# interactiveaudiolab/emphases

Hardware: AMD Instinct MI355X
Metric: utterances/s (10 s @16 kHz) whole-node (higher is better)
Workload: dtype f32; 1 GPU; 64 synthetic 10 s 16 kHz utterances per GPU, conv config, random word alignments, ragged batch with per-utterance (B=1) semantics (BASELINE.json configs[1]); utterances_per_gpu=64, frames_per_gpu=64000, words_per_gpu=1882, conv_tile=64, launch=hipGraph replay, batches_in_flight=2, parallelism=utterance-sharded x1, exchange=none (one rank)

## Files before the change

### emphases_amd/csrc/decoder.hip

```cpp
#include <math.h>
#include <stdint.h>

#include <type_traits>

#include "common.h"

namespace emph {

typedef float f32x4 __attribute__((ext_vector_type(4)));

constexpr int kWindow = 64;
constexpr int kLeadCols = 4;
constexpr int kActStride = 80;

__device__ __forceinline__ float activate_word(float x, int act) {
    switch (act) {
        case EMPH_ACT_RELU: return fmaxf(x, 0.f);
        case EMPH_ACT_GELU: return 0.5f * x * (1.f + erff(x * 0.70710678118654752440f));
        case EMPH_ACT_SILU: return x / (1.f + expf(-x));
        case EMPH_ACT_LEAKY_RELU: return x > 0.f ? x : 0.01f * x;
        default: return x;
    }
}

#ifndef EMPH_DECODER_LOADERS
#define EMPH_DECODER_LOADERS 4
#endif
constexpr int kLoaderWaves = EMPH_DECODER_LOADERS;

template <int KS, int MT>
__global__ __launch_bounds__(64 * (8 + kLoaderWaves)) void word_decoder_kernel(
    const float* __restrict__ x, int64_t ldx, const int32_t* __restrict__ tiles,
    int block, int halo, int channels, const float* __restrict__ packs,
    const float* __restrict__ biases, int layers, int act, int chunk_trips,
    const float* __restrict__ out_weight, const float* __restrict__ out_bias,
    int out_kernel, int post, float* __restrict__ logits, float* __restrict__ scores) {
    extern __shared__ __align__(16) float lds[];
    const int m_tiles = channels >> 4;
    const int threads = blockDim.x;
    const int waves = threads >> 6;
    const int compute_waves = waves - kLoaderWaves;
    const int buffer_floats = channels * kActStride;
    float* partial = lds + 2 * channels * kActStride;
    float* bias_lds = partial + waves * kWindow;
    float* out_lds = bias_lds + layers * channels;
    float* ring = lds + ((2 * channels * kActStride + waves * kWindow + layers * channels +
                          channels * out_kernel + 1 + 3) & ~3);
    const int lane = threadIdx.x & 63;
    const int wave = __builtin_amdgcn_readfirstlane(threadIdx.x >> 6);
    const int kk = lane >> 4;
    const int col = lane & 15;

    const Tile span = load_tile(tiles, blockIdx.x);
    const int reach = 32 - halo;
    const bool halves = span.count > 32 && span.count <= 2 * reach;
    const bool second = halves && span.first != 0;
    const bool single = span.count <= kWindow && !halves;
    if (single && span.first != 0) return;
    const int half = (span.count + 1) >> 1;
    const int first_out = halves ? (second ? half : 0) : span.first;
    const int last_out = halves   ? (second ? span.count : half)
                         : single ? span.count
                                  : min(span.first + block, span.count);
    const int start = halves ? (second ? span.count - 32 : 0) : single ? 0 : span.first - halo;
    const bool narrow = halves || (single && span.count <= 32);

    constexpr int HALO = (KS - 1) / 2;
    constexpr int kTripFloats = 4 * KS;
    const int trips = channels >> 4;
    const int trip_floats = m_tiles * 64 * kTripFloats;
    const int chunks_per_layer = (trips + chunk_trips - 1) / chunk_trips;
    const int total_chunks = layers * chunks_per_layer;
    const int chunk_floats = chunk_trips * trip_floats;
    auto request = [&](int q) {
        const int layer = q / chunks_per_layer;
        const int first = (q - layer * chunks_per_layer) * chunk_trips;
        const int quads = min(chunk_trips, trips - first) * (trip_floats >> 2);
        const float* source =
            packs + (static_cast<int64_t>(layer) * trips + first) * trip_floats;
        float* target = ring + (q & 1) * chunk_floats;
        for (int base = 64 * (wave - compute_waves); base < quads;
             base += 64 * kLoaderWaves)
            __builtin_amdgcn_global_load_lds(
                (const __attribute__((address_space(1))) void*)(source + 4 * (base + lane)),
                (__attribute__((address_space(3))) void*)(target + 4 * base), 16, 0, 0);
    };
    const bool loader = wave >= compute_waves;
    if (total_chunks > 0 && loader) request(0);

    for (int index = threadIdx.x; index < channels * (kActStride / 4); index += threads) {
        const int c = index / (kActStride / 4);
        const int quad = index - c * (kActStride / 4);
        float4 value = make_float4(0.f, 0.f, 0.f, 0.f);
        const int p = 4 * quad - kLeadCols;
        if (p >= 0 && p < kWindow) {
            const int word = start + p;
            const float* source = x + static_cast<int64_t>(c) * ldx + span.offset + word;
            if (word >= 0 && word + 3 < span.count &&
                (reinterpret_cast<uintptr_t>(source) & 15) == 0) {
                value = *reinterpret_cast<const float4*>(source);
            } else {
                if (word >= 0 && word < span.count) value.x = source[0];
                if (word + 1 >= 0 && word + 1 < span.count) value.y = source[1];
                if (word + 2 >= 0 && word + 2 < span.count) value.z = source[2];
                if (word + 3 >= 0 && word + 3 < span.count) value.w = source[3];
            }
        }
        reinterpret_cast<float4*>(lds)[index] = value;
        reinterpret_cast<float4*>(lds + buffer_floats)[index] =
            make_float4(0.f, 0.f, 0.f, 0.f);
    }
    for (int index = threadIdx.x; index < layers * channels; index += threads)
        bias_lds[index] = biases[index];
    for (int index = threadIdx.x; index <= channels * out_kernel; index += threads)
        out_lds[index] = index < channels * out_kernel ? out_weight[index] : out_bias[0];

    if (loader) {
        for (int q = 0; q < total_chunks; ++q) {
            __builtin_amdgcn_s_waitcnt(0x0F70);
            __syncthreads();
            if (q + 1 < total_chunks) request(q + 1);
        }
    }

    const int n_tile = narrow ? (wave & 1) : (wave & 3);
    const int part = narrow ? (wave >> 1) : (wave >> 2);
    const int split = (m_tiles + 1) >> 1;
    const int m_begin = narrow ? (m_tiles * part + 3) >> 2 : (part ? split : 0);
    const int m_end = narrow ? (m_tiles * (part + 1) + 3) >> 2 : (part ? m_tiles : split);
    const int m_count = m_end - m_begin;
    auto run_layers = [&](auto count_tag) {
        constexpr int COUNT = decltype(count_tag)::value;
        int buffer = 0;
        for (int layer = 0; layer < layers; ++layer) {
            const float* source = lds + buffer * buffer_floats;
            float* target = lds + (buffer ^ 1) * buffer_floats;
// ... 41 lines not shown
                    for (int tap = 0; tap < KS; ++tap)
#pragma unroll
                        for (int i = 0; i < COUNT; ++i) {
                            acc[i] = __builtin_amdgcn_mfma_f32_16x16x4f32(
                                a[i][(t * KS + tap) >> 2][(t * KS + tap) & 3], b[t][tap],
                                acc[i], 0, 0, 0);
                        }
#pragma unroll
                for (int k = 0; k < (COUNT + 4) * KS; ++k) {
                    __builtin_amdgcn_sched_group_barrier(0x008, 1, 0);
                    __builtin_amdgcn_sched_group_barrier(0x100, 1, 0);
                }
                __builtin_amdgcn_sched_barrier(0);
            };
            __syncthreads();
            if (kTwoSets) {
                issue(a_set[0], b_set[0], 0);
                for (int trip = 0; trip < trips; trip += 2) {
                    step(a_set[0], b_set[0], a_set[kTwoSets], b_set[kTwoSets], trip);
                    if (trip + 1 < trips)
                        step(a_set[kTwoSets], b_set[kTwoSets], a_set[0], b_set[0], trip + 1);
                }
            } else {
                for (int trip = 0; trip < trips; ++trip)
                    step(a_set[0], b_set[0], a_set[0], b_set[0], trip);
            }
            const float* bias = bias_lds + layer * channels + 16 * m_begin + 4 * kk;
            const int p = 16 * n_tile + col;
            const int word = start + p;
            const bool inside = word >= 0 && word < span.count;
            f32x4 value[COUNT];
#pragma unroll
            for (int i = 0; i < COUNT; ++i)
                value[i] = acc[i] + *reinterpret_cast<const f32x4*>(bias + 16 * i);
#define EMPH_APPLY(EXPRESSION)                                   \
    _Pragma("unroll") for (int i = 0; i < COUNT; ++i)            \
// ... 6 lines not shown
                case EMPH_ACT_GELU:
                    EMPH_APPLY(0.5f * v * (1.f + erff(v * 0.70710678118654752440f)));
                    break;
                case EMPH_ACT_SILU: EMPH_APPLY(v / (1.f + expf(-v))); break;
                case EMPH_ACT_LEAKY_RELU: EMPH_APPLY(v > 0.f ? v : 0.01f * v); break;
                default: break;
            }
#undef EMPH_APPLY
#pragma unroll
            for (int i = 0; i < COUNT; ++i)
#pragma unroll
                for (int r = 0; r < 4; ++r) {
                    const int c = 16 * (m_begin + i) + 4 * kk + r;
                    target[c * kActStride + kLeadCols + p] = inside ? value[i][r] : 0.f;
                }
            buffer ^= 1;
        }
    };
    if (!loader) {
        if (m_count >= 4 && MT >= 4) run_layers(std::integral_constant<int, MT >= 4 ? 4 : 1>{});
        else if (m_count == 3) run_layers(std::integral_constant<int, 3>{});
        else if (m_count == 2) run_layers(std::integral_constant<int, 2>{});
        else if (m_count == 1) run_layers(std::integral_constant<int, 1>{});
        else
            for (int q = 0; q < total_chunks; ++q) __syncthreads();
    }
    int current = layers & 1;
    __syncthreads();

    {
        const float* source = lds + current * buffer_floats;
        const int halo_out = (out_kernel - 1) / 2;
        float sum = 0.f;
        for (int c = wave; c < channels && !loader; c += compute_waves)
// ... 6 lines not shown
            float total = out_lds[channels * out_kernel];
            for (int w = 0; w < compute_waves; ++w) total += partial[w * kWindow + lane];
            const int word = start + lane;
            if (word >= first_out && word < last_out) {
                const int64_t column = span.offset + word;
                if (logits != nullptr) logits[column] = total;
                if (scores != nullptr) {
                    float value = total;
                    if (post == EMPH_POST_SIGMOID) value = 1.f / (1.f + expf(-total));
                    if (post == EMPH_POST_CLAMP01) value = fminf(fmaxf(total, 0.f), 1.f);
                    scores[column] = value;
                }
            }
        }
    }
}

}

using namespace emph;

extern "C" {

int64_t emph_word_decoder_pack_size(int32_t channels, int32_t kernel_size) {
    return static_cast<int64_t>(channels) * channels * kernel_size;
}

int emph_word_decoder_pack(const float* host_weight, int32_t channels, int32_t kernel_size,
                           float* host_pack) {
    EMPH_REQUIRE(host_weight && host_pack, EMPH_EINVAL,
// ... 46 lines not shown
    for (int segment = 0; segment < segments; ++segment) {
        const int64_t count = host_counts[segment];
        if (count <= 0) continue;
        if (count > 32 && count <= 2 * (32 - halo)) {
            emit(segment, 0);
            emit(segment, (count + 1) / 2);
        } else if (count <= kWindow) {
            emit(segment, 0);
        } else {
            for (int64_t first = 0; first < count; first += block) emit(segment, first);
        }
    }
    return total;
}

int emph_word_decoder(const float* x, int64_t ldx, const int32_t* tiles,
                      int32_t n_tiles, int32_t channels, const float* packs,
                      const float* biases, int32_t layers, int32_t kernel_size,
                      int32_t activation, const float* out_weight,
                      const float* out_bias, int32_t out_kernel_size, int32_t post,
                      float* logits, float* scores, void* stream) {
    if (n_tiles == 0) return EMPH_OK;
    EMPH_REQUIRE(x && tiles && out_weight && out_bias, EMPH_EINVAL,
                 "emph_word_decoder: null pointer");
    EMPH_REQUIRE(layers == 0 || (packs && biases), EMPH_EINVAL,
                 "emph_word_decoder: decoder weights are null");
    EMPH_REQUIRE(layers >= 0 && layers <= 16, EMPH_ERANGE,
                 "emph_word_decoder: %d layers", layers);
    EMPH_REQUIRE(channels >= 16 && channels <= 128 && channels % 16 == 0, EMPH_ERANGE,
                 "emph_word_decoder: channels %d not a multiple of 16 in 16..128",
                 channels);
    EMPH_REQUIRE(kernel_size == 1 || kernel_size == 3 || kernel_size == 5, EMPH_ERANGE,
                 "emph_word_decoder: kernel_size %d not in {1,3,5}", kernel_size);
    EMPH_REQUIRE(out_kernel_size >= 1 && out_kernel_size <= 7 && (out_kernel_size & 1),
                 EMPH_ERANGE, "emph_word_decoder: out_kernel_size %d", out_kernel_size);
    const int block = emph_word_decoder_block(layers, kernel_size, out_kernel_size);
    EMPH_REQUIRE(block >= 16, EMPH_ERANGE,
                 "emph_word_decoder: receptive field too wide for a 64-word window");
    const int halo = (kWindow - block) / 2;
    const int m_tiles = channels / 16;
    const int threads = 64 * (8 + kLoaderWaves);
    const size_t fixed_floats = (2 * channels * kActStride + (threads / 64) * kWindow +
                                 layers * channels + channels * out_kernel_size + 1 + 3) & ~3;
    size_t ring_budget = 156 * 1024 - fixed_floats * sizeof(float);
    const int trips = channels / 16;
    const size_t trip_bytes = static_cast<size_t>(m_tiles) * 64 * 4 * kernel_size * sizeof(float);
    int chunk_trips = static_cast<int>(ring_budget / 2 / trip_bytes);
    EMPH_REQUIRE(chunk_trips >= 1, EMPH_ERANGE,
                 "emph_word_decoder: no LDS left for the weight ring (%d channels, %d layers)",
                 channels, layers);
    if (chunk_trips > trips) chunk_trips = trips;
    const int pieces = (trips + chunk_trips - 1) / chunk_trips;
    chunk_trips = (trips + pieces - 1) / pieces;
    const size_t lds = fixed_floats * sizeof(float) + 2 * chunk_trips * trip_bytes;
    hipStream_t s = static_cast<hipStream_t>(stream);
#define EMPH_WORDS(KS)                                                              \
    do {                                                                            \
        auto kernel = m_tiles <= 6 ? word_decoder_kernel<KS, 3>                     \
                                   : word_decoder_kernel<KS, 4>;                    \
        static LdsReservation reserved[2];                                                     \
        if (int status = reserve_lds(reserved[m_tiles <= 6], reinterpret_cast<const void*>(kernel), lds,\
                                     "emph_word_decoder"))                                     \
            return status;                                                                     \
        EMPH_LAUNCH(kernel, dim3(n_tiles), dim3(threads), lds, s, x, ldx,     \
                           tiles, block, halo, channels, packs, biases, layers,      \
                           activation, chunk_trips, out_weight, out_bias,            \
                           out_kernel_size, post, logits, scores);                   \
    } while (0)
    switch (kernel_size) {
        case 1: EMPH_WORDS(1); break;
        case 3: EMPH_WORDS(3); break;
        default: EMPH_WORDS(5); break;
    }
#undef EMPH_WORDS
    return check_launch("emph_word_decoder");
}

}
```

### emphases_amd/csrc/forward.hip

```cpp
#include "common.h"

using namespace emph;

namespace emph {
__global__ __launch_bounds__(64) void launch_probe_kernel() {}
}

extern "C" {

int emph_launch_probe(void* stream) {
    EMPH_LAUNCH(launch_probe_kernel, dim3(1), dim3(64), 0, static_cast<hipStream_t>(stream));
    return check_launch("emph_launch_probe");
}

int64_t emph_prominence_workspace_floats(int32_t features, int32_t channels,
                                         int64_t ld_frames, int64_t ld_words,
                                         int32_t n_slots) {
    return (static_cast<int64_t>(features) + 2 * channels) * ld_frames +
           static_cast<int64_t>(channels) * (ld_words + n_slots);
}

int emph_prominence_forward(const emph_conv_model* model, const void* audio,
                            int32_t audio_format, const int64_t* seg,
                            const int32_t* frontend_tiles,
// ... 39 lines not shown
                 "emph_prominence_forward: word_sums needs conv_variant 1 and a sum / average "
                 "reduction");

    int status = emph_logmel(audio, audio_format, seg, frontend_tiles, n_frontend_tiles, m.table,
                             m.mel_start, m.mel_count, m.mel_offset, m.mel_values, m.mel_nnz,
                             features, ld_frames, 0, -1, nullptr, nullptr, m.normalize, stream);
    if (status) return status;
    auto conv = [&](const float* in, float* out, const float* pack, const float* bias, int c_in,
                    int activation) {
        return quad ? emph_conv1d_winograd4(in, ld_frames, out, ld_frames, pack, bias, c_in, c,
                                            activation, frame_tiles, n_frame_tiles, stream)
                    : emph_conv1d_winograd(in, ld_frames, out, ld_frames, pack, bias, c_in, c,
                                           activation, frame_tiles, n_frame_tiles, tile_n,
                                           stream);
    };
    const int64_t pack_floats =
        quad ? emph_conv_winograd4_pack_size(c, c) : emph_conv_winograd_pack_size(c, c);
    const bool stack = conv_spans != nullptr && quad && c == 80 && m.features == 80 &&
                       m.encoder_packs == m.input_pack + pack_floats &&
                       m.encoder_biases == m.input_bias + c &&
                       (m.activation == EMPH_ACT_RELU || m.activation == EMPH_ACT_NONE);
    if (stack) {
        const bool composed = m.compose != nullptr && m.encoder_layers >= 1;
        const int skip = composed ? 1 : 0;
        const int total = 1 + m.encoder_layers - skip;
        const int most = emph_conv_stack_max_layers();
        const int groups = (total + most - 1) / most;
        float* buffers[2] = {current, other};
        const float* in = features;
        int done = 0;
// ... 13 lines not shown
                               n_conv_spans, to_sums ? word_sums->slot_map : nullptr, stream)
                         : emph_conv1d_stack(in, ld_frames, out, to_sums ? c : ld_frames, packs,
                                             biases, size, relu, conv_spans, n_conv_spans,
                                             to_sums ? word_sums->slot_map : nullptr, stream);
            if (status) return status;
            in = out;
            done += size;
        }
        current = const_cast<float*>(in);
        status = fold ? emph_word_sums(sums, c, word_sums->terms, word_sums->first,
                                       word_sums->lengths, words, ld_words, c, ld_words,
                                       m.reduction, stream)
                      : emph_segment_reduce(current, ld_frames, bounds, words, ld_words, c, seg,
                                            word_segment, ld_words, m.reduction, stream);
        if (status) return status;
        return emph_word_decoder(words, ld_words, word_tiles, n_word_tiles, c, m.decoder_packs,
                                 m.decoder_biases, m.decoder_layers, m.decoder_kernel_size,
                                 m.activation, m.out_weight, m.out_bias, m.decoder_kernel_size,
                                 m.post, logits, scores, stream);
    }
    status = conv(features, current, m.input_pack, m.input_bias, m.features, EMPH_ACT_NONE);
    if (status) return status;
    for (int layer = 0; layer < m.encoder_layers; ++layer) {
        if (fold && layer == m.encoder_layers - 1) {
            status = emph_conv1d_winograd4_word_sums(
                current, ld_frames, sums, c, m.encoder_packs + layer * pack_floats,
                m.encoder_biases + static_cast<int64_t>(layer) * c, c, c, m.activation,
                frame_tiles, n_frame_tiles, word_sums->slot_map, stream);
            if (status) return status;
            break;
        }
        status = conv(current, other, m.encoder_packs + layer * pack_floats,
                      m.encoder_biases + static_cast<int64_t>(layer) * c, c, m.activation);
        if (status) return status;
        float* swap = current;
        current = other;
        other = swap;
    }
    status = fold ? emph_word_sums(sums, c, word_sums->terms, word_sums->first,
                                   word_sums->lengths, words, ld_words, c, ld_words,
                                   m.reduction, stream)
                  : emph_segment_reduce(current, ld_frames, bounds, words, ld_words, c, seg,
                                        word_segment, ld_words, m.reduction, stream);
    if (status) return status;
    return emph_word_decoder(words, ld_words, word_tiles, n_word_tiles, c, m.decoder_packs,
                             m.decoder_biases, m.decoder_layers, m.decoder_kernel_size,
                             m.activation, m.out_weight, m.out_bias, m.decoder_kernel_size,
                             m.post, logits, scores, stream);
}

}
```

### emphases_amd/engine.py

```python
import contextlib
import functools
import os
import ctypes
import threading

import numpy as np
import torch

from . import config as cfg
from . import melbasis
from . import runtime
from . import weights as weights_module

FRONTEND_BLOCK = None
PRECISIONS = {'f32': (0, 0, 0), 'bf16x3': (2, 32, 3), 'bf16x3_fast': (2, 32, 2),
              'bf16x6': (0, 3, 3)}
ATTENTION_BLOCK = 64
ATTENTION_GROUP = 256
GROUPED_FROM = ATTENTION_GROUP // 2
FUSED_WORDS = 64
EVERYTHING = 1 << 30
SHORT, LONG = (0, GROUPED_FROM - 1), (GROUPED_FROM, EVERYTHING)
FEW_WORDS, MANY_WORDS = (0, FUSED_WORDS), (FUSED_WORDS + 1, EVERYTHING)
WORD_TILE = 16
# ... 122 lines not shown
        self.mel_values = to(basis.values)
        self.mel_nnz = int(basis.values.size)
        self.a_weights = to(a_weighting())

        self.input_layer = _Conv(
            state['input_layer.weight'], state['input_layer.bias'], dev,
            winograd)
        self.frame_encoder = self._stack('frame_encoder')
        self.word_decoder = self._stack('word_decoder') \
            if config.has_decoder else None
        self.output_weight = to(state['output_layer.weight'])
        self.output_bias = to(state['output_layer.bias'])
        self.fused_words = config.architecture == 'convolution' or \
            not config.has_decoder
        self.word_block = WORD_TILE
        if self.fused_words:
            layers = self.word_decoder if config.has_decoder else []
            self.decoder_layers = len(layers)
            self.decoder_packs = torch.from_numpy(np.concatenate([
                runtime.word_decoder_pack(l.weight) for l in layers])).to(dev) \
                if layers else None
            self.decoder_biases = torch.cat([l.bias for l in layers]) \
                if layers else None
            self.word_block = int(self.lib.emph_word_decoder_block(
                self.decoder_layers, config.decoder_kernel_size,
                config.decoder_kernel_size))
            self.decoder_tiles = (runtime.AXIS_DECODER, (
                self.decoder_layers, config.decoder_kernel_size,
                config.decoder_kernel_size))
        if config.architecture == 'transformer':
            self.position = to(weights_module.positional_encoding(
                cfg.MAX_POSITIONS, config.channels))
            self.position_rows = self.position.t().contiguous()
        self.word_transformer = None
        if config.architecture == 'transformer' and config.has_decoder and \
                config.channels in (64, 80) and config.heads == 2 and all(
                    tuple(state[f'word_decoder.model.layers.{i}.{name}.weight']
                          .shape) == (config.channels, config.channels)
# ... 88 lines not shown
            post=runtime.POSTPROCESS[config.loss],
            normalize=int(config.normalize), mel_nnz=self.mel_nnz,
            conv_variant=int(self.quad),
            table=pointer(self.table), mel_start=pointer(self.mel_start),
            mel_count=pointer(self.mel_count),
            mel_offset=pointer(self.mel_offset),
            mel_values=pointer(self.mel_values),
            input_pack=pointer(input_pack),
            input_bias=pointer(input_bias),
            encoder_packs=pointer(self._encoder_packs),
            encoder_biases=pointer(self._encoder_biases),
            decoder_packs=pointer(self.decoder_packs),
            decoder_biases=pointer(self.decoder_biases),
            out_weight=pointer(self.output_weight),
            out_bias=pointer(self.output_bias),
            compose=pointer(self._compose_pack if self.stack else None))

    def _stack(self, prefix):
        config, state, dev = self.config, self.state, self.device
        layers = []
        if config.architecture == 'convolution':
            for i in range(config.layers):
                layers.append(_Conv(
                    state[f'{prefix}.{2 * i}.weight'],
                    state[f'{prefix}.{2 * i}.bias'], dev,
                    self.winograd and prefix == 'frame_encoder'))
            return layers
        channels = config.channels
        to = lambda a: torch.from_numpy(np.ascontiguousarray(a)).to(dev)
        for i in range(config.layers):
            p = f'{prefix}.model.layers.{i}.'
# ... 889 lines not shown
            logits[at:at + size].copy_(
                part_logits[batch.LEAD:batch.LEAD + size])
        return scores, logits

    def _word_stage(self, wa, plan, meta, logits, scores):
        config = self.config
        channels = config.channels
        ld_w = plan.ld_words
        words = runtime.AXIS_WORDS
        table = meta['table'][0]
        if self.fused_words:
            tiles, size = meta[('tiles',) + self.decoder_tiles]
            with self._timed('word_decoder', 2. * channels * (
                    channels * config.decoder_kernel_size * self.decoder_layers
                    + config.decoder_kernel_size) * plan.total_words):
                runtime.check(self.lib.emph_word_decoder(
                    wa.data_ptr(), ld_w, tiles.data_ptr(),
                    size // runtime.TILE_FIELDS, channels,
                    None if self.decoder_packs is None
                    else self.decoder_packs.data_ptr(),
                    None if self.decoder_biases is None
                    else self.decoder_biases.data_ptr(),
                    self.decoder_layers, config.decoder_kernel_size,
                    runtime.ACTIVATIONS[config.activation],
                    self.output_weight.data_ptr(), self.output_bias.data_ptr(),
                    config.decoder_kernel_size,
                    runtime.POSTPROCESS[config.loss], logits.data_ptr(),
                    scores.data_ptr(), runtime.stream()), 'emph_word_decoder')
            return scores, logits
        wb = self._buffer('words_b', channels, ld_w)
        decoded = self._stack_forward(
            self.word_decoder, wa, wb, ld_w, plan, meta, words,
            self.word_block, 'words')
        with self._timed('output_layer'):
            runtime.check(self.lib.emph_output_layer(
# ... 79 lines not shown
```

### emphases_amd/runtime.py

```python
import ctypes
import os

import numpy as np
import torch

HERE = os.path.dirname(os.path.abspath(__file__))
LIBRARY_PATH = os.path.join(HERE, 'libemphases_hip.so')
ABI_VERSION = 39

SEG_FIELDS = 8
TILE_FIELDS = 4
(SEG_AUDIO_OFF, SEG_AUDIO_LEN, SEG_START, SEG_LENGTH, SEG_FRAME_OFF,
 SEG_FRAMES, SEG_WORD_OFF, SEG_WORDS) = range(8)
AXIS_FRAMES, AXIS_WORDS = 0, 1
AXIS_DECODER = 2
ACTIVATIONS = {None: 0, 'none': 0, 'relu': 1, 'gelu': 2, 'silu': 3,
               'leaky_relu': 4}
REDUCTIONS = {'sum': 0, 'average': 1, 'max': 2, 'center': 3}
POSTPROCESS = {None: 0, 'bce': 1, 'mse': 2}
BCE_FORMS = {'bce': 0, 'mse': 1}
AUDIO_F32, AUDIO_PCM16 = 0, 1
SPREAD_IDENTITY, SPREAD_LOG2 = 0, 1
(METRIC_COUNT, METRIC_BCE, METRIC_SQUARED_ERROR, METRIC_COVARIANCE,
 METRIC_SUM_PREDICTED, METRIC_SUMSQ_PREDICTED, METRIC_SUM_TARGET,
# ... 126 lines not shown
        _ptr, _ptr, _i64, _ptr, _ptr]),
    'emph_plan_word_sums': (_i64, [
        _ptr, _ptr, _ptr, _i32, _ptr, _ptr, _i64, _ptr, _i64, _i64, _i64,
        _ptr, _ptr, _ptr, _ptr, _i64, _ptr]),
    'emph_gather_columns': (_c.c_int, [
        _ptr, _i64, _ptr, _i64, _i32, _ptr, _i32, _ptr]),
    'emph_collate': (_c.c_int, [
        _ptr, _i64, _ptr, _i64, _ptr, _i32, _i32, _i64, _i64, _ptr, _ptr,
        _ptr]),
    'emph_unpack_rows': (_c.c_int, [_ptr, _i64, _ptr, _i32, _ptr, _ptr]),
    'emph_word_decoder_block': (_i32, [_i32, _i32, _i32]),
    'emph_word_decoder_tiles': (_i32, [_ptr, _ptr, _i32, _i32, _i32, _i32, _ptr]),
    'emph_word_decoder_pack_size': (_i64, [_i32, _i32]),
    'emph_word_decoder_pack': (_c.c_int, [_ptr, _i32, _i32, _ptr]),
    'emph_word_decoder': (_c.c_int, [
        _ptr, _i64, _ptr, _i32, _i32, _ptr, _ptr, _i32, _i32, _i32, _ptr, _ptr,
        _i32, _i32, _ptr, _ptr, _ptr]),
    'emph_add_position': (_c.c_int, [
        _ptr, _i64, _ptr, _i32, _i32, _ptr, _i32, _i32, _ptr]),
    'emph_attention': (_c.c_int, [
        _ptr, _ptr, _ptr, _i64, _i32, _i32, _ptr, _i32, _i32, _ptr, _ptr]),
    'emph_split_kv_bytes': (_i64, [_i64, _i32, _i32, _i32, _i32]),
    'emph_split_kv': (_c.c_int, [
        _ptr, _ptr, _i64, _i32, _i32, _ptr, _i32, _i32, _i32, _ptr, _ptr]),
    'emph_attention_split': (_c.c_int, [
        _ptr, _ptr, _ptr, _i64, _i32, _i32, _ptr, _i32, _i32, _ptr, _i32,
        _ptr]),
    'emph_word_transformer_pack_size': (_i64, [_i32, _i32]),
    'emph_word_transformer_pack': (_c.c_int, [_ptr] * 12 + [_i32, _i32, _ptr]),
    'emph_word_transformer': (_c.c_int, [
# ... 184 lines not shown
                    dtype=np.float32)
    check(lib.emph_word_transformer_pack(
        *[array.ctypes.data for array in arrays], channels, heads,
        pack.ctypes.data), 'emph_word_transformer_pack')
    return pack


class ConvModel(_c.Structure):
    _fields_ = [(name, _i32) for name in (
        'channels', 'features', 'encoder_layers', 'decoder_layers',
        'decoder_kernel_size', 'activation', 'reduction', 'post',
        'normalize', 'mel_nnz', 'conv_variant')] + [(name, _ptr) for name in (
            'table', 'mel_start', 'mel_count', 'mel_offset', 'mel_values',
            'input_pack', 'input_bias', 'encoder_packs', 'encoder_biases',
            'decoder_packs', 'decoder_biases', 'out_weight', 'out_bias',
            'compose')]


class WordSumTables(_c.Structure):
    _fields_ = [(name, _ptr) for name in (
        'slot_map', 'terms', 'first', 'lengths')] + [('n_slots', _i32)]


def word_decoder_pack(weight):
    lib = library()
    weight = np.ascontiguousarray(weight, dtype=np.float32)
    channels, c_in, kernel_size = weight.shape
    assert channels == c_in
    pack = np.zeros(
        lib.emph_word_decoder_pack_size(channels, kernel_size),
        dtype=np.float32)
    check(lib.emph_word_decoder_pack(
        weight.ctypes.data, channels, kernel_size, pack.ctypes.data),
        'emph_word_decoder_pack')
    return pack


def conv_compose_pack(w0, b0, w1, b1):
    lib = library()
    arrays = [np.ascontiguousarray(a, dtype=np.float32)
              for a in (w0, b0, w1, b1)]
    assert arrays[0].shape == arrays[2].shape == (80, 80, 3)
    assert arrays[1].shape == arrays[3].shape == (80,)
    pack = np.zeros(lib.emph_conv_compose_pack_size(), dtype=np.float32)
    check(lib.emph_conv_compose_pack(
        *[a.ctypes.data for a in arrays], pack.ctypes.data),
        'emph_conv_compose_pack')
    return pack


def conv_split_pack(weight):
    lib = library()
# ... 69 lines not shown
```

### include/emphases_hip.h

```cpp
#ifndef EMPHASES_HIP_H
#define EMPHASES_HIP_H

#include <stdint.h>

#ifdef __cplusplus
extern "C" {
#endif

#define EMPH_ABI_VERSION 39

enum {
    EMPH_SEG_AUDIO_OFF = 0,
    EMPH_SEG_AUDIO_LEN = 1,
    EMPH_SEG_START = 2,
    EMPH_SEG_LENGTH = 3,
    EMPH_SEG_FRAME_OFF = 4,
    EMPH_SEG_FRAMES = 5,
    EMPH_SEG_WORD_OFF = 6,
    EMPH_SEG_WORDS = 7,
    EMPH_SEG_FIELDS = 8
};

enum { EMPH_AXIS_FRAMES = 0, EMPH_AXIS_WORDS = 1 };

// ... 240 lines not shown
int32_t emph_word_decoder_tiles(const int64_t* host_counts,
                                const int64_t* host_offsets, int32_t segments,
                                int32_t layers, int32_t kernel_size,
                                int32_t out_kernel_size, int32_t* host_tiles);

int64_t emph_word_decoder_pack_size(int32_t channels, int32_t kernel_size);
int emph_word_decoder_pack(const float* host_weight, int32_t channels,
                           int32_t kernel_size, float* host_pack);

int emph_word_decoder(const float* x, int64_t ldx, const int32_t* tiles,
                      int32_t n_tiles, int32_t channels, const float* packs,
                      const float* biases, int32_t layers, int32_t kernel_size,
                      int32_t activation, const float* out_weight,
                      const float* out_bias, int32_t out_kernel_size,
                      int32_t post, float* logits, float* scores, void* stream);


int emph_add_position(float* x, int64_t ldx, const float* table,
                      int32_t channels, int32_t max_positions,
                      const int32_t* tiles, int32_t n_tiles, int32_t tile_n,
                      void* stream);

int emph_attention(const float* qk, const float* v, float* out, int64_t ld,
                   int32_t channels, int32_t heads, const int32_t* tiles,
                   int32_t n_tiles, int32_t tile_n, const int32_t* key_counts,
                   void* stream);

int64_t emph_split_kv_bytes(int64_t ld, int32_t n_segments, int32_t channels,
                            int32_t heads, int32_t pieces);
int emph_split_kv(const float* qk, const float* v, int64_t ld, int32_t channels,
// ... 140 lines not shown
    int32_t conv_variant;
    const float* table;
    const int32_t* mel_start;
    const int32_t* mel_count;
    const int32_t* mel_offset;
    const float* mel_values;
    const float* input_pack;
    const float* input_bias;
    const float* encoder_packs;
    const float* encoder_biases;
    const float* decoder_packs;
    const float* decoder_biases;
    const float* out_weight;
    const float* out_bias;
    const float* compose;
} emph_conv_model;

typedef struct emph_word_sum_tables {
    const int32_t* slot_map;
    const int32_t* terms;
    const int32_t* first;
    const int32_t* lengths;
    int32_t n_slots;
} emph_word_sum_tables;

int64_t emph_prominence_workspace_floats(int32_t features, int32_t channels,
                                         int64_t ld_frames, int64_t ld_words,
                                         int32_t n_slots);

int emph_prominence_forward(const emph_conv_model* model, const void* audio,
// ... 88 lines not shown
```

Baseline: 465,600 utterances/s.

## Add Winograd F(2,3) path for the 80-channel kernel-3 word decoder

Adds a Winograd F(2,3) variant of the word decoder kernel. Each of four wave groups computes one transformed point with MFMA, and the outputs are combined through an LDS scratch buffer with bias and activation applied. Weights are pre-transformed on the host into a new pack, and the LDS weight ring gains deeper prefetch with explicit vmcnt waits. The aim is to cut decoder MFMA work per layer, at the cost of extra LDS scratch, more barriers and a reduction step. The path is enabled by default for 80 channels with kernel size 3.

New measurement: 470,100 utterances/s (median of 6 runs). About the same (+1.0%).

```diff
diff --git a/emphases_amd/csrc/decoder.hip b/emphases_amd/csrc/decoder.hip
--- a/emphases_amd/csrc/decoder.hip
+++ b/emphases_amd/csrc/decoder.hip
@@ -12,6 +12,8 @@
 constexpr int kWindow = 64;
 constexpr int kLeadCols = 4;
 constexpr int kActStride = 80;
+constexpr int kF23Jobs = 20;
+constexpr int kF23ScratchFloats = kF23Jobs * 256;
 
 __device__ __forceinline__ float activate_word(float x, int act) {
     switch (act) {
@@ -23,12 +25,17 @@
     }
 }
 
+#ifndef EMPH_STAMP
+#define EMPH_STAMP(slot)
+#endif
 #ifndef EMPH_DECODER_LOADERS
 #define EMPH_DECODER_LOADERS 4
 #endif
 constexpr int kLoaderWaves = EMPH_DECODER_LOADERS;
-
-template <int KS, int MT>
+constexpr int kF23Requests = 20 % kLoaderWaves == 0 ? 20 / kLoaderWaves : 0;
+static_assert(2 * kF23Requests < 64, "s_waitcnt vmcnt immediate");
+
+template <int KS, int MT, bool F23 = false>
 __global__ __launch_bounds__(64 * (8 + kLoaderWaves)) void word_decoder_kernel(
     const float* __restrict__ x, int64_t ldx, const int32_t* __restrict__ tiles,
     int block, int halo, int channels, const float* __restrict__ packs,
@@ -44,13 +51,15 @@
     float* partial = lds + 2 * channels * kActStride;
     float* bias_lds = partial + waves * kWindow;
     float* out_lds = bias_lds + layers * channels;
-    float* ring = lds + ((2 * channels * kActStride + waves * kWindow + layers * channels +
-                          channels * out_kernel + 1 + 3) & ~3);
+    float* scratch = lds + ((2 * channels * kActStride + waves * kWindow + layers * channels +
+                             channels * out_kernel + 1 + 3) & ~3);
+    float* ring = scratch + (F23 ? kF23ScratchFloats : 0);
     const int lane = threadIdx.x & 63;
     const int wave = __builtin_amdgcn_readfirstlane(threadIdx.x >> 6);
     const int kk = lane >> 4;
     const int col = lane & 15;
 
+    EMPH_STAMP(0);
     const Tile span = load_tile(tiles, blockIdx.x);
     const int reach = 32 - halo;
     const bool halves = span.count > 32 && span.count <= 2 * reach;
@@ -66,9 +75,12 @@
     const bool narrow = halves || (single && span.count <= 32);
 
     constexpr int HALO = (KS - 1) / 2;
-    constexpr int kTripFloats = 4 * KS;
+    constexpr int kTripFloats = F23 ? 16 : 4 * KS;
     const int trips = channels >> 4;
     const int trip_floats = m_tiles * 64 * kTripFloats;
+    const int slots = F23 ? chunk_trips : 2;
+    if (F23) chunk_trips = 1;
+    const int ahead = slots - 2;
     const int chunks_per_layer = (trips + chunk_trips - 1) / chunk_trips;
     const int total_chunks = layers * chunks_per_layer;
     const int chunk_floats = chunk_trips * trip_floats;
@@ -78,7 +90,7 @@
         const int quads = min(chunk_trips, trips - first) * (trip_floats >> 2);
         const float* source =
             packs + (static_cast<int64_t>(layer) * trips + first) * trip_floats;
-        float* target = ring + (q & 1) * chunk_floats;
+        float* target = ring + (F23 ? q % slots : q & 1) * chunk_floats;
         for (int base = 64 * (wave - compute_waves); base < quads;
              base += 64 * kLoaderWaves)
             __builtin_amdgcn_global_load_lds(
@@ -86,7 +98,8 @@
                 (__attribute__((address_space(3))) void*)(target + 4 * base), 16, 0, 0);
     };
     const bool loader = wave >= compute_waves;
-    if (total_chunks > 0 && loader) request(0);
+    if (loader)
+        for (int q = 0; q <= ahead && q < total_chunks; ++q) request(q);
 
     for (int index = threadIdx.x; index < channels * (kActStride / 4); index += threads) {
         const int c = index / (kActStride / 4);
@@ -114,12 +127,31 @@
         bias_lds[index] = biases[index];
     for (int index = threadIdx.x; index <= channels * out_kernel; index += threads)
         out_lds[index] = index < channels * out_kernel ? out_weight[index] : out_bias[0];
+    EMPH_STAMP(1);
 
     if (loader) {
         for (int q = 0; q < total_chunks; ++q) {
-            __builtin_amdgcn_s_waitcnt(0x0F70);
-            __syncthreads();
-            if (q + 1 < total_chunks) request(q + 1);
+            if constexpr (F23) {
+                const int behind = min(ahead, total_chunks - 1 - q);
+                if (behind >= 2) {
+                    asm volatile("s_waitcnt vmcnt(%0) lgkmcnt(0)" ::"n"(2 * kF23Requests) : "memory");
+                } else if (behind == 1) {
+                    asm volatile("s_waitcnt vmcnt(%0) lgkmcnt(0)" ::"n"(kF23Requests) : "memory");
+                } else {
+                    asm volatile("s_waitcnt vmcnt(0) lgkmcnt(0)" ::: "memory");
+                }
+                __builtin_amdgcn_s_barrier();
+                asm volatile("" ::: "memory");
+            } else {
+                __builtin_amdgcn_s_waitcnt(0x0F70);
+                __syncthreads();
+            }
+            if (q + 1 + ahead < total_chunks) request(q + 1 + ahead);
+            if (F23 && (q + 1) % chunks_per_layer == 0)
+                for (int i = 0; i < (narrow ? 1 : 3); ++i) {
+                    asm volatile("" ::: "memory");
+                    __builtin_amdgcn_s_barrier();
+                }
         }
     }
 
@@ -191,12 +223,15 @@
                 __builtin_amdgcn_sched_barrier(0);
             };
             __syncthreads();
+            if (layer == 1) EMPH_STAMP(10);
             if (kTwoSets) {
                 issue(a_set[0], b_set[0], 0);
                 for (int trip = 0; trip < trips; trip += 2) {
                     step(a_set[0], b_set[0], a_set[kTwoSets], b_set[kTwoSets], trip);
+                    if (layer == 1 && trip < 5) EMPH_STAMP(11 + trip);
                     if (trip + 1 < trips)
                         step(a_set[kTwoSets], b_set[kTwoSets], a_set[0], b_set[0], trip + 1);
+                    if (layer == 1 && trip < 4) EMPH_STAMP(12 + trip);
                 }
             } else {
                 for (int trip = 0; trip < trips; ++trip)
@@ -233,10 +268,147 @@
                     const int c = 16 * (m_begin + i) + 4 * kk + r;
                     target[c * kActStride + kLeadCols + p] = inside ? value[i][r] : 0.f;
                 }
+            if (layer < 6) EMPH_STAMP(3 + layer);
             buffer ^= 1;
         }
     };
-    if (!loader) {
+    auto run_layers_f23 = [&](auto count_tag) {
+        constexpr int COUNT = decltype(count_tag)::value;
+        constexpr int kStepFloats = kF23Jobs * 64;
+        const int point = wave & 3;
+        const int tile = narrow ? 0 : wave >> 2;
+        const int m_first = narrow && wave >= 4 ? 3 : 0;
+        const int first = point == 0 ? 0 : point == 2 ? 2 : 1;
+        const int second = point == 2 ? 1 : point == 3 ? 3 : 2;
+        const float sign = point == 1 ? 1.f : -1.f;
+        const int rounds = narrow ? 1 : 2;
+        int buffer = 0;
+        for (int layer = 0; layer < layers; ++layer) {
+            const float* source = lds + buffer * buffer_floats;
+            float* target = lds + (buffer ^ 1) * buffer_floats;
+            f32x4 acc[COUNT];
+#pragma unroll
+            for (int i = 0; i < COUNT; ++i) acc[i] = f32x4{0.f, 0.f, 0.f, 0.f};
+            float a_set[2][4][COUNT];
+            float b_set[2][4][2];
+            auto issue = [&](float (&a_out)[4][COUNT], float (&b_out)[4][2], int trip) {
+                const int piece = trip / chunk_trips;
+                const int q = layer * chunks_per_layer + piece;
+                const float* fragment = ring + (q % slots) * chunk_floats +
+                                        (trip - piece * chunk_trips) * trip_floats +
+                                        (point * 5 + m_first) * 64 + lane;
+                const float* b_base = source + (16 * trip + kk) * kActStride + kLeadCols +
+                                      32 * tile + 2 * col - 1;
+#pragma unroll
+                for (int s = 0; s < 4; ++s)
+#pragma unroll
+                    for (int i = 0; i < COUNT; ++i)
+                        a_out[s][i] = fragment[s * kStepFloats + i * 64];
+#pragma unroll
+                for (int s = 0; s < 4; ++s) {
+                    b_out[s][0] = b_base[4 * s * kActStride + first];
+                    b_out[s][1] = b_base[4 * s * kActStride + second];
+                }
+            };
+            auto step = [&](float (&a)[4][COUNT], float (&b)[4][2], float (&a_out)[4][COUNT],
+                            float (&b_out)[4][2], int trip) {
+                const int next = min(trip + 1, trips - 1);
+                if (trip + 1 < trips && (trip + 1) % chunk_trips == 0)
+                    __syncthreads();
+                __builtin_amdgcn_sched_barrier(0);
+                issue(a_out, b_out, next);
+#pragma unroll
+                for (int s = 0; s < 4; ++s) {
+                    const float v = fmaf(sign, b[s][1], b[s][0]);
+#pragma unroll
+                    for (int i = 0; i < COUNT; ++i)
+                        acc[i] = __builtin_amdgcn_mfma_f32_16x16x4f32(a[s][i], v, acc[i], 0, 0, 0);
+                }
+#pragma unroll
+                for (int k = 0; k < 8; ++k) {
+                    __builtin_amdgcn_sched_group_barrier(0x008, 1, 0);
+                    __builtin_amdgcn_sched_group_barrier(0x100, 2, 0);
+                }
+#pragma unroll
+                for (int k = 8; k < 4 * COUNT; ++k) {
+                    __builtin_amdgcn_sched_group_barrier(0x008, 1, 0);
+                    __builtin_amdgcn_sched_group_barrier(0x100, 1, 0);
+                }
+                __builtin_amdgcn_sched_barrier(0);
+            };
+            __syncthreads();
+            if (layer == 1) EMPH_STAMP(10);
+            issue(a_set[0], b_set[0], 0);
+            for (int trip = 0; trip < trips; trip += 2) {
+                step(a_set[0], b_set[0], a_set[1], b_set[1], trip);
+                if (layer == 1 && trip < 5) EMPH_STAMP(11 + trip);
+                if (trip + 1 < trips) step(a_set[1], b_set[1], a_set[0], b_set[0], trip + 1);
+                if (layer == 1 && trip < 4) EMPH_STAMP(12 + trip);
+            }
+            for (int round = 0; round < rounds; ++round) {
+                if (tile == round) {
+#pragma unroll
+                    for (int i = 0; i < COUNT; ++i)
+#pragma unroll
+                        for (int r = 0; r < 4; ++r)
+                            scratch[((point * 5 + m_first + i) * 4 + r) * 64 + lane] = acc[i][r];
+                }
+                __syncthreads();
+                float value[3][2];
+#pragma unroll
+                for (int j = 0; j < 3; ++j) {
+                    const int item = min(wave + 8 * j, kF23Jobs - 1);
+                    const float m0 = scratch[(0 * kF23Jobs + item) * 64 + lane];
+                    const float m1 = scratch[(1 * kF23Jobs + item) * 64 + lane];
+                    const float m2 = scratch[(2 * kF23Jobs + item) * 64 + lane];
+                    const float m3 = scratch[(3 * kF23Jobs + item) * 64 + lane];
+                    const float bias =
+                        bias_lds[layer * channels + 16 * (item >> 2) + 4 * kk + (item & 3)];
+                    value[j][0] = ((m0 + m1) + m2) + bias;
+                    value[j][1] = ((m1 - m2) - m3) + bias;
+                }
+#define EMPH_APPLY(EXPRESSION)                                   \
+    _Pragma("unroll") for (int j = 0; j < 3; ++j)                \
+        _Pragma("unroll") for (int e = 0; e < 2; ++e) {          \
+            const float v = value[j][e];                         \
+            value[j][e] = (EXPRESSION);                          \
+        }
+                switch (act) {
+                    case EMPH_ACT_RELU: EMPH_APPLY(v < 0.f ? 0.f : v); break;
+                    case EMPH_ACT_GELU:
+                        EMPH_APPLY(0.5f * v * (1.f + erff(v * 0.70710678118654752440f)));
+                        break;
+                    case EMPH_ACT_SILU: EMPH_APPLY(v / (1.f + expf(-v))); break;
+                    case EMPH_ACT_LEAKY_RELU: EMPH_APPLY(v > 0.f ? v : 0.01f * v); break;
+                    default: break;
+                }
+#undef EMPH_APPLY
+                const int p = 32 * round + 2 * col;
+                const int word = start + p;
+#pragma unroll
+                for (int j = 0; j < 3; ++j) {
+                    const int item = wave + 8 * j;
+                    if (item < kF23Jobs) {
+                        const int c = 16 * (item >> 2) + 4 * kk + (item & 3);
+                        float2 pair;
+                        pair.x = word >= 0 && word < span.count ? value[j][0] : 0.f;
+                        pair.y = word + 1 >= 0 && word + 1 < span.count ? value[j][1] : 0.f;
+                        *reinterpret_cast<float2*>(target + c * kActStride + kLeadCols + p) = pair;
+                    }
+                }
+                if (round + 1 < rounds) __syncthreads();
+            }
+            if (layer < 6) EMPH_STAMP(3 + layer);
+            buffer ^= 1;
+        }
+    };
+    if constexpr (F23) {
+        if (!loader) {
+            if (!narrow) run_layers_f23(std::integral_constant<int, 5>{});
+            else if (wave < 4) run_layers_f23(std::integral_constant<int, 3>{});
+            else run_layers_f23(std::integral_constant<int, 2>{});
+        }
+    } else if (!loader) {
         if (m_count >= 4 && MT >= 4) run_layers(std::integral_constant<int, MT >= 4 ? 4 : 1>{});
         else if (m_count == 3) run_layers(std::integral_constant<int, 3>{});
         else if (m_count == 2) run_layers(std::integral_constant<int, 2>{});
@@ -273,6 +445,7 @@
             }
         }
     }
+    EMPH_STAMP(9);
 }
 
 }
@@ -349,66 +522,129 @@
     return total;
 }
 
+int64_t emph_word_decoder_pack_f23_size(int32_t channels) {
+    return static_cast<int64_t>(channels) * channels * 4;
+}
+
+int emph_word_decoder_pack_f23(const float* host_weight, int32_t channels, float* host_pack) {
+    EMPH_REQUIRE(host_weight && host_pack, EMPH_EINVAL,
+                 "emph_word_decoder_pack_f23: null pointer");
+    EMPH_REQUIRE(channels == 80, EMPH_ERANGE,
+                 "emph_word_decoder_pack_f23: channels %d, not 80", channels);
+    const int m_tiles = channels / 16, steps = channels / 4;
+    for (int step = 0; step < steps; ++step)
+        for (int m = 0; m < m_tiles; ++m)
+            for (int lane = 0; lane < 64; ++lane) {
+                const int co = 16 * m + (lane & 15);
+                const int ci = 4 * step + (lane >> 4);
+                const float* g = host_weight + (static_cast<int64_t>(co) * channels + ci) * 3;
+                const double g0 = g[0], g1 = g[1], g2 = g[2];
+                const double u[4] = {g0, 0.5 * (g0 + g1 + g2), 0.5 * (g0 - g1 + g2), g2};
+                for (int point = 0; point < 4; ++point)
+                    host_pack[((static_cast<int64_t>(step) * 4 + point) * m_tiles + m) * 64 +
+                              lane] = static_cast<float>(u[point]);
+            }
+    return EMPH_OK;
+}
+
+static int launch_word_decoder(const char* name, bool f23, const float* x, int64_t ldx,
+                               const int32_t* tiles, int32_t n_tiles, int32_t channels,
+                               const float* packs, const float* biases, int32_t layers,
+                               int32_t kernel_size, int32_t activation, const float* out_weight,
+                               const float* out_bias, int32_t out_kernel_size, int32_t post,
+                               float* logits, float* scores, void* stream) {
+    if (n_tiles == 0) return EMPH_OK;
+    EMPH_REQUIRE(x && tiles && out_weight && out_bias, EMPH_EINVAL, "%s: null pointer", name);
+    EMPH_REQUIRE(layers == 0 || (packs && biases), EMPH_EINVAL,
+                 "%s: decoder weights are null", name);
+    EMPH_REQUIRE(layers >= 0 && layers <= 16, EMPH_ERANGE, "%s: %d layers", name, layers);
+    EMPH_REQUIRE(channels >= 16 && channels <= 128 && channels % 16 == 0, EMPH_ERANGE,
+                 "%s: channels %d not a multiple of 16 in 16..128", name, channels);
+    EMPH_REQUIRE(kernel_size == 1 || kernel_size == 3 || kernel_size == 5, EMPH_ERANGE,
+                 "%s: kernel_size %d not in {1,3,5}", name, kernel_size);
+    EMPH_REQUIRE(!f23 || (channels == 80 && kernel_size == 3), EMPH_ERANGE,
+                 "%s: %d channels, kernel_size %d: F(2,3) is for 80 and 3", name, channels,
+                 kernel_size);
+    EMPH_REQUIRE(out_kernel_size >= 1 && out_kernel_size <= 7 && (out_kernel_size & 1),
+                 EMPH_ERANGE, "%s: out_kernel_size %d", name, out_kernel_size);
+    const int block = emph_word_decoder_block(layers, kernel_size, out_kernel_size);
+    EMPH_REQUIRE(block >= 16, EMPH_ERANGE,
+                 "%s: receptive field too wide for a 64-word window", name);
+    const int halo = (kWindow - block) / 2;
+    const int m_tiles = channels / 16;
+    const int threads = 64 * (8 + kLoaderWaves);
+    const size_t fixed_floats = ((2 * channels * kActStride + (threads / 64) * kWindow +
+                                  layers * channels + channels * out_kernel_size + 1 + 3) & ~3) +
+                                (f23 ? kF23ScratchFloats : 0);
+    EMPH_REQUIRE(fixed_floats * sizeof(float) < 156 * 1024, EMPH_ERANGE,
+                 "%s: no LDS left for the weight ring (%d channels, %d layers)", name, channels,
+                 layers);
+    size_t ring_budget = 156 * 1024 - fixed_floats * sizeof(float);
+    const int trips = channels / 16;
+    const size_t trip_bytes =
+        static_cast<size_t>(m_tiles) * 64 * (f23 ? 16 : 4 * kernel_size) * sizeof(float);
+    int chunk_trips = static_cast<int>(ring_budget / 2 / trip_bytes);
+    EMPH_REQUIRE(chunk_trips >= 1, EMPH_ERANGE,
+                 "%s: no LDS left for the weight ring (%d channels, %d layers)", name, channels,
+                 layers);
+    if (chunk_trips > trips) chunk_trips = trips;
+    const int pieces = (trips + chunk_trips - 1) / chunk_trips;
+    chunk_trips = (trips + pieces - 1) / pieces;
+    const int slots =
+        !f23 ? 2 : kF23Requests == 0 ? 2 : static_cast<int>(ring_budget / trip_bytes) >= 4 ? 4 : 2;
+    if (f23) chunk_trips = slots;
+    const size_t lds =
+        fixed_floats * sizeof(float) + (f23 ? slots : 2 * chunk_trips) * trip_bytes;
+    hipStream_t s = static_cast<hipStream_t>(stream);
+#define EMPH_WORDS_LAUNCH(KERNEL, SLOT)                                                        \
+    do {                                                                                       \
+        auto kernel = KERNEL;                                                                  \
+        static LdsReservation reserved[2];                                                     \
+        if (int status = reserve_lds(reserved[SLOT], reinterpret_cast<const void*>(kernel),    \
+                                     lds, name))                                               \
+            return status;                                                                     \
+        EMPH_LAUNCH(kernel, dim3(n_tiles), dim3(threads), lds, s, x, ldx, tiles, block, halo,  \
+                    channels, packs, biases, layers, activation, chunk_trips, out_weight,      \
+                    out_bias, out_kernel_size, post, logits, scores);                          \
+    } while (0)
+#define EMPH_WORDS(KS)                                                                         \
+    EMPH_WORDS_LAUNCH((m_tiles <= 6 ? word_decoder_kernel<KS, 3> : word_decoder_kernel<KS, 4>), \
+                      m_tiles <= 6)
+    if (f23) {
+        EMPH_WORDS_LAUNCH((word_decoder_kernel<3, 3, true>), 0);
+    } else {
+        switch (kernel_size) {
+            case 1: EMPH_WORDS(1); break;
+            case 3: EMPH_WORDS(3); break;
+            default: EMPH_WORDS(5); break;
+        }
+    }
+#undef EMPH_WORDS
+#undef EMPH_WORDS_LAUNCH
+    return check_launch(name);
+}
+
 int emph_word_decoder(const float* x, int64_t ldx, const int32_t* tiles,
                       int32_t n_tiles, int32_t channels, const float* packs,
                       const float* biases, int32_t layers, int32_t kernel_size,
                       int32_t activation, const float* out_weight,
                       const float* out_bias, int32_t out_kernel_size, int32_t post,
                       float* logits, float* scores, void* stream) {
-    if (n_tiles == 0) return EMPH_OK;
-    EMPH_REQUIRE(x && tiles && out_weight && out_bias, EMPH_EINVAL,
-                 "emph_word_decoder: null pointer");
-    EMPH_REQUIRE(layers == 0 || (packs && biases), EMPH_EINVAL,
-                 "emph_word_decoder: decoder weights are null");
-    EMPH_REQUIRE(layers >= 0 && layers <= 16, EMPH_ERANGE,
-                 "emph_word_decoder: %d layers", layers);
-    EMPH_REQUIRE(channels >= 16 && channels <= 128 && channels % 16 == 0, EMPH_ERANGE,
-                 "emph_word_decoder: channels %d not a multiple of 16 in 16..128",
-                 channels);
-    EMPH_REQUIRE(kernel_size == 1 || kernel_size == 3 || kernel_size == 5, EMPH_ERANGE,
-                 "emph_word_decoder: kernel_size %d not in {1,3,5}", kernel_size);
-    EMPH_REQUIRE(out_kernel_size >= 1 && out_kernel_size <= 7 && (out_kernel_size & 1),
-                 EMPH_ERANGE, "emph_word_decoder: out_kernel_size %d", out_kernel_size);
-    const int block = emph_word_decoder_block(layers, kernel_size, out_kernel_size);
-    EMPH_REQUIRE(block >= 16, EMPH_ERANGE,
-                 "emph_word_decoder: receptive field too wide for a 64-word window");
-    const int halo = (kWindow - block) / 2;
-    const int m_tiles = channels / 16;
-    const int threads = 64 * (8 + kLoaderWaves);
-    const size_t fixed_floats = (2 * channels * kActStride + (threads / 64) * kWindow +
-                                 layers * channels + channels * out_kernel_size + 1 + 3) & ~3;
-    size_t ring_budget = 156 * 1024 - fixed_floats * sizeof(float);
-    const int trips = channels / 16;
-    const size_t trip_bytes = static_cast<size_t>(m_tiles) * 64 * 4 * kernel_size * sizeof(float);
-    int chunk_trips = static_cast<int>(ring_budget / 2 / trip_bytes);
-    EMPH_REQUIRE(chunk_trips >= 1, EMPH_ERANGE,
-                 "emph_word_decoder: no LDS left for the weight ring (%d channels, %d layers)",
-                 channels, layers);
-    if (chunk_trips > trips) chunk_trips = trips;
-    const int pieces = (trips + chunk_trips - 1) / chunk_trips;
-    chunk_trips = (trips + pieces - 1) / pieces;
-    const size_t lds = fixed_floats * sizeof(float) + 2 * chunk_trips * trip_bytes;
-    hipStream_t s = static_cast<hipStream_t>(stream);
-#define EMPH_WORDS(KS)                                                              \
-    do {                                                                            \
-        auto kernel = m_tiles <= 6 ? word_decoder_kernel<KS, 3>                     \
-                                   : word_decoder_kernel<KS, 4>;                    \
-        static LdsReservation reserved[2];                                                     \
-        if (int status = reserve_lds(reserved[m_tiles <= 6], reinterpret_cast<const void*>(kernel), lds,\
-                                     "emph_word_decoder"))                                     \
-            return status;                                                                     \
-        EMPH_LAUNCH(kernel, dim3(n_tiles), dim3(threads), lds, s, x, ldx,     \
-                           tiles, block, halo, channels, packs, biases, layers,      \
-                           activation, chunk_trips, out_weight, out_bias,            \
-                           out_kernel_size, post, logits, scores);                   \
-    } while (0)
-    switch (kernel_size) {
-        case 1: EMPH_WORDS(1); break;
-        case 3: EMPH_WORDS(3); break;
-        default: EMPH_WORDS(5); break;
-    }
-#undef EMPH_WORDS
-    return check_launch("emph_word_decoder");
-}
-
-}
+    return launch_word_decoder("emph_word_decoder", false, x, ldx, tiles, n_tiles, channels,
+                               packs, biases, layers, kernel_size, activation, out_weight,
+                               out_bias, out_kernel_size, post, logits, scores, stream);
+}
+
+int emph_word_decoder_f23(const float* x, int64_t ldx, const int32_t* tiles,
+                          int32_t n_tiles, int32_t channels, const float* packs,
+                          const float* biases, int32_t layers, int32_t kernel_size,
+                          int32_t activation, const float* out_weight,
+                          const float* out_bias, int32_t out_kernel_size, int32_t post,
+                          float* logits, float* scores, void* stream) {
+    return launch_word_decoder("emph_word_decoder_f23", true, x, ldx, tiles, n_tiles,
+                               channels, packs, biases, layers, kernel_size, activation,
+                               out_weight, out_bias, out_kernel_size, post, logits, scores,
+                               stream);
+}
+
+}
diff --git a/emphases_amd/csrc/forward.hip b/emphases_amd/csrc/forward.hip
--- a/emphases_amd/csrc/forward.hip
+++ b/emphases_amd/csrc/forward.hip
@@ -77,6 +77,9 @@
                                            activation, frame_tiles, n_frame_tiles, tile_n,
                                            stream);
     };
+    const bool f23 = m.decoder_f23 != nullptr && m.decoder_layers > 0;
+    const auto decoder = f23 ? emph_word_decoder_f23 : emph_word_decoder;
+    const float* decoder_packs = f23 ? m.decoder_f23 : m.decoder_packs;
     const int64_t pack_floats =
         quad ? emph_conv_winograd4_pack_size(c, c) : emph_conv_winograd_pack_size(c, c);
     const bool stack = conv_spans != nullptr && quad && c == 80 && m.features == 80 &&
@@ -120,10 +123,10 @@
                       : emph_segment_reduce(current, ld_frames, bounds, words, ld_words, c, seg,
                                             word_segment, ld_words, m.reduction, stream);
         if (status) return status;
-        return emph_word_decoder(words, ld_words, word_tiles, n_word_tiles, c, m.decoder_packs,
-                                 m.decoder_biases, m.decoder_layers, m.decoder_kernel_size,
-                                 m.activation, m.out_weight, m.out_bias, m.decoder_kernel_size,
-                                 m.post, logits, scores, stream);
+        return decoder(words, ld_words, word_tiles, n_word_tiles, c, decoder_packs,
+                       m.decoder_biases, m.decoder_layers, m.decoder_kernel_size,
+                       m.activation, m.out_weight, m.out_bias, m.decoder_kernel_size,
+                       m.post, logits, scores, stream);
     }
     status = conv(features, current, m.input_pack, m.input_bias, m.features, EMPH_ACT_NONE);
     if (status) return status;
@@ -149,10 +152,10 @@
                   : emph_segment_reduce(current, ld_frames, bounds, words, ld_words, c, seg,
                                         word_segment, ld_words, m.reduction, stream);
     if (status) return status;
-    return emph_word_decoder(words, ld_words, word_tiles, n_word_tiles, c, m.decoder_packs,
-                             m.decoder_biases, m.decoder_layers, m.decoder_kernel_size,
-                             m.activation, m.out_weight, m.out_bias, m.decoder_kernel_size,
-                             m.post, logits, scores, stream);
+    return decoder(words, ld_words, word_tiles, n_word_tiles, c, decoder_packs,
+                   m.decoder_biases, m.decoder_layers, m.decoder_kernel_size, m.activation,
+                   m.out_weight, m.out_bias, m.decoder_kernel_size, m.post, logits, scores,
+                   stream);
 }
 
 }
diff --git a/emphases_amd/engine.py b/emphases_amd/engine.py
--- a/emphases_amd/engine.py
+++ b/emphases_amd/engine.py
@@ -160,6 +160,7 @@
         self.fused_words = config.architecture == 'convolution' or \
             not config.has_decoder
         self.word_block = WORD_TILE
+        self.decoder_winograd, self.decoder_packs_f23 = False, None
         if self.fused_words:
             layers = self.word_decoder if config.has_decoder else []
             self.decoder_layers = len(layers)
@@ -168,6 +169,15 @@
                 if layers else None
             self.decoder_biases = torch.cat([l.bias for l in layers]) \
                 if layers else None
+            self.decoder_winograd = bool(
+                layers and config.channels == 80 and
+                config.decoder_kernel_size == 3 and
+                config.activation != 'leaky_relu' and
+                config.downsample_method != 'center' and
+                os.environ.get('EMPHASES_DECODER_WINOGRAD', '1') != '0')
+            self.decoder_packs_f23 = torch.from_numpy(np.concatenate([
+                runtime.word_decoder_pack_f23(l.weight) for l in layers])).to(
+                    dev) if self.decoder_winograd else None
             self.word_block = int(self.lib.emph_word_decoder_block(
                 self.decoder_layers, config.decoder_kernel_size,
                 config.decoder_kernel_size))
@@ -286,7 +296,8 @@
             decoder_biases=pointer(self.decoder_biases),
             out_weight=pointer(self.output_weight),
             out_bias=pointer(self.output_bias),
-            compose=pointer(self._compose_pack if self.stack else None))
+            compose=pointer(self._compose_pack if self.stack else None),
+            decoder_f23=pointer(self.decoder_packs_f23))
 
     def _stack(self, prefix):
         config, state, dev = self.config, self.state, self.device
@@ -1206,11 +1217,14 @@
             with self._timed('word_decoder', 2. * channels * (
                     channels * config.decoder_kernel_size * self.decoder_layers
                     + config.decoder_kernel_size) * plan.total_words):
-                runtime.check(self.lib.emph_word_decoder(
+                packs = self.decoder_packs_f23 if self.decoder_winograd \
+                    else self.decoder_packs
+                decoder = self.lib.emph_word_decoder_f23 \
+                    if self.decoder_winograd else self.lib.emph_word_decoder
+                runtime.check(decoder(
                     wa.data_ptr(), ld_w, tiles.data_ptr(),
                     size // runtime.TILE_FIELDS, channels,
-                    None if self.decoder_packs is None
-                    else self.decoder_packs.data_ptr(),
+                    None if packs is None else packs.data_ptr(),
                     None if self.decoder_biases is None
                     else self.decoder_biases.data_ptr(),
                     self.decoder_layers, config.decoder_kernel_size,
diff --git a/emphases_amd/runtime.py b/emphases_amd/runtime.py
--- a/emphases_amd/runtime.py
+++ b/emphases_amd/runtime.py
@@ -6,7 +6,7 @@
 
 HERE = os.path.dirname(os.path.abspath(__file__))
 LIBRARY_PATH = os.path.join(HERE, 'libemphases_hip.so')
-ABI_VERSION = 39
+ABI_VERSION = 40
 
 SEG_FIELDS = 8
 TILE_FIELDS = 4
@@ -164,6 +164,11 @@
     'emph_word_decoder_pack_size': (_i64, [_i32, _i32]),
     'emph_word_decoder_pack': (_c.c_int, [_ptr, _i32, _i32, _ptr]),
     'emph_word_decoder': (_c.c_int, [
+        _ptr, _i64, _ptr, _i32, _i32, _ptr, _ptr, _i32, _i32, _i32, _ptr, _ptr,
+        _i32, _i32, _ptr, _ptr, _ptr]),
+    'emph_word_decoder_pack_f23_size': (_i64, [_i32]),
+    'emph_word_decoder_pack_f23': (_c.c_int, [_ptr, _i32, _ptr]),
+    'emph_word_decoder_f23': (_c.c_int, [
         _ptr, _i64, _ptr, _i32, _i32, _ptr, _ptr, _i32, _i32, _i32, _ptr, _ptr,
         _i32, _i32, _ptr, _ptr, _ptr]),
     'emph_add_position': (_c.c_int, [
@@ -378,7 +383,7 @@
             'table', 'mel_start', 'mel_count', 'mel_offset', 'mel_values',
             'input_pack', 'input_bias', 'encoder_packs', 'encoder_biases',
             'decoder_packs', 'decoder_biases', 'out_weight', 'out_bias',
-            'compose')]
+            'compose', 'decoder_f23')]
 
 
 class WordSumTables(_c.Structure):
@@ -400,6 +405,19 @@
     return pack
 
 
+def word_decoder_pack_f23(weight):
+    lib = library()
+    weight = np.ascontiguousarray(weight, dtype=np.float32)
+    channels, c_in, kernel_size = weight.shape
+    assert channels == c_in and kernel_size == 3
+    pack = np.zeros(
+        lib.emph_word_decoder_pack_f23_size(channels), dtype=np.float32)
+    check(lib.emph_word_decoder_pack_f23(
+        weight.ctypes.data, channels, pack.ctypes.data),
+        'emph_word_decoder_pack_f23')
+    return pack
+
+
 def conv_compose_pack(w0, b0, w1, b1):
     lib = library()
     arrays = [np.ascontiguousarray(a, dtype=np.float32)
diff --git a/include/emphases_hip.h b/include/emphases_hip.h
--- a/include/emphases_hip.h
+++ b/include/emphases_hip.h
@@ -7,7 +7,7 @@
 extern "C" {
 #endif
 
-#define EMPH_ABI_VERSION 39
+#define EMPH_ABI_VERSION 40
 
 enum {
     EMPH_SEG_AUDIO_OFF = 0,
@@ -278,6 +278,17 @@
                       int32_t activation, const float* out_weight,
                       const float* out_bias, int32_t out_kernel_size,
                       int32_t post, float* logits, float* scores, void* stream);
+
+int64_t emph_word_decoder_pack_f23_size(int32_t channels);
+int emph_word_decoder_pack_f23(const float* host_weight, int32_t channels,
+                               float* host_pack);
+int emph_word_decoder_f23(const float* x, int64_t ldx, const int32_t* tiles,
+                          int32_t n_tiles, int32_t channels, const float* packs,
+                          const float* biases, int32_t layers,
+                          int32_t kernel_size, int32_t activation,
+                          const float* out_weight, const float* out_bias,
+                          int32_t out_kernel_size, int32_t post, float* logits,
+                          float* scores, void* stream);
 
 
 int emph_add_position(float* x, int64_t ldx, const float* table,
@@ -448,6 +459,7 @@
     const float* out_weight;
     const float* out_bias;
     const float* compose;
+    const float* decoder_f23;
 } emph_conv_model;
 
 typedef struct emph_word_sum_tables {
```
